# buwantaiji/FermiFlow

Hardware: NVIDIA B200
Metric: VMC walker-updates/s (sample+E_loc+grad) N=20 (higher is better)
Workload: dtype f64

## Files before the change

### fermiflow_b200/csrc/capi.cu

```cuda
#define FF_RADIAL_TABLE_KERNELS
#include "capi_flow.h"
#include "ff_adjoint.cuh"
#include "ff_pgrad_binned.cuh"
#include "ff_misc.cuh"
#include "ff_metro_reg.cuh"
#include "ff_observables.cuh"

namespace ffc {


thread_local char g_err[512] = "";

int fail(int code, const char* fmt, ...) {
    va_list ap;
    va_start(ap, fmt);
    vsnprintf(g_err, sizeof(g_err), fmt, ap);
    va_end(ap);
    return code;
}

int cuda_fail(cudaError_t e, const char* what) {
    return fail((int)e, "%s: %s", what, cudaGetErrorString(e));
}

const char* const kOptNames[] = {
    "no_table", "no_w_balance", "no_rt_cache", "flow_warp_fill", "flow_cta", "flow_big", "eloc_generic", "slater_cta",
    "metropolis_kernel", "adjoint_cta", "pgrad_direct", "pgrad_tile", "pgrad_fixed_range", "adjoint_no_prefetch", "finale_cta",
    "metropolis_no_split"};
static_assert(sizeof(kOptNames) / sizeof(kOptNames[0]) == OPT_COUNT, "one name per option");
std::atomic<int> g_opt[OPT_COUNT];
std::atomic<long long> g_launches{0};

DevInfo dev_info() {
    static thread_local DevInfo di[16];
    int dev = 0;
    cudaGetDevice(&dev);
    DevInfo& d = di[dev & 15];
    if (!d.ok) {
        cudaDeviceGetAttribute(&d.sms, cudaDevAttrMultiProcessorCount, dev);
        cudaDeviceGetAttribute(&d.smem_optin, cudaDevAttrMaxSharedMemoryPerBlockOptin, dev);
        cudaDeviceGetAttribute(&d.smem_sm, cudaDevAttrMaxSharedMemoryPerMultiprocessor, dev);
        cudaDeviceGetAttribute(&d.smem_reserved, cudaDevAttrReservedSharedMemoryPerBlock, dev);
        d.ok = true;
    }
    return d;
}

int check_model(const ff_model* m) {
    if (!m) return fail(-1, "model is null");
    const int n = m->n_up + m->n_dn;
    if (m->n_up < 0 || m->n_dn < 0 || n < 1) return fail(-1, "bad particle numbers %d/%d", m->n_up, m->n_dn);
    if (n > 200) return fail(-1, "n = %d particles exceeds the supported 200", n);
    if (m->H_eta < 1 || m->H_mu < 0) return fail(-1, "bad hidden sizes");
    if (m->nsteps < 1) return fail(-1, "nsteps must be >= 1");
    if (!m->eta_w1 || !m->eta_b1 || !m->eta_w2) return fail(-1, "eta parameters missing");
    if (m->H_mu > 0 && (!m->mu_w1 || !m->mu_b1 || !m->mu_w2)) return fail(-1, "mu parameters missing");
    return 0;
}

int RadialTables::build(const ff_model* m, cudaStream_t stream, ff::FlowArgs& a) {
    a.rt_eta = nullptr; a.rt_mu = nullptr;
    if (opt(OPT_NO_TABLE)) return 0;
    st = stream;
    {
        static thread_local bool pool_ready[16] = {};
        int dev = 0;
        cudaGetDevice(&dev);
        if (!pool_ready[dev & 15]) {
            cudaMemPool_t pool;
            if (cudaDeviceGetDefaultMemPool(&pool, dev) == cudaSuccess) {
                unsigned long long keep = 64ull << 20;
                cudaMemPoolSetAttribute(pool, cudaMemPoolAttrReleaseThreshold, &keep);
            }
            pool_ready[dev & 15] = true;
        }
    }
    const size_t per = ff::radial_table_doubles();
    FF_CUDA(cudaMallocAsync((void**)&buf, 2 * per * sizeof(double), st));
    ff::RadialBuildArgs b{};
    b.w1[0] = m->eta_w1; b.b1[0] = m->eta_b1; b.w2[0] = m->eta_w2; b.H[0] = m->H_eta; b.table[0] = buf;
    b.w1[1] = m->mu_w1; b.b1[1] = m->mu_b1; b.w2[1] = m->mu_w2; b.H[1] = m->H_mu; b.table[1] = m->H_mu > 0 ? buf + per : nullptr;
    ff::radial_table_build_kernel<<<dim3(ff::kRtMaxNodes / 128, 2), 128, 0, st>>>(b);
    FF_LAUNCHED();
    ff::radial_table_check_kernel<<<dim3(1, 2), 128, 0, st>>>(b.table[0], b.table[1]);
    FF_LAUNCHED();
    a.rt_eta = b.table[0]; a.rt_mu = b.table[1];
    return 0;
}

}

using namespace ffc;

extern "C" {

int ff_version(void) { return 200; }

long long ff_launch_count(void) { return g_launches.load(std::memory_order_relaxed); }

int ff_set_option(const char* name, int value) {
    if (!name) return fail(-1, "ff_set_option: null name");
    for (int k = 0; k < OPT_COUNT; ++k)
        if (strcmp(name, kOptNames[k]) == 0) { g_opt[k].store(value, std::memory_order_relaxed); return 0; }
    return fail(-1, "ff_set_option: unknown option '%s'", name);
}
int ff_get_option(const char* name, int* value) {
    if (!name || !value) return fail(-1, "ff_get_option: null argument");
    for (int k = 0; k < OPT_COUNT; ++k)
        if (strcmp(name, kOptNames[k]) == 0) { *value = opt((Opt)k); return 0; }
    return fail(-1, "ff_get_option: unknown option '%s'", name);
}
const char* ff_last_error(void) { return g_err; }

int ff_stash_sizes(const ff_model* m, long long B, long long* ny, long long* nc) {
    if (int e = check_model(m)) return e;
    const long long n = m->n_up + m->n_dn, NS = 4LL * m->nsteps;
    const long long P = n * (n - 1) / 2 + (m->H_mu > 0 ? n : 0);
    if (ny) *ny = B * NS * 2 * n;
    if (nc) *nc = B * NS * P * 3;
    return 0;
}

int ff_cnf_generate(const ff_model* m, const double* z, long long B, int reverse, double* x, void* stream) {
    if (int e = check_model(m)) return e;
    if (B < 0 || (B > 0 && (!z || !x))) return fail(-1, "ff_cnf_generate: null buffer");
    ff::FlowArgs a{};
    int threads; size_t smem;
    if (int e = plan_flow(ff::MODE_V, m, a, threads, smem)) return e;
    a.ta = reverse ? m->t1 : m->t0; a.tb = reverse ? m->t0 : m->t1;
    a.B = B; a.x_in = z; a.y_out = x;
    RadialTables rt;
    if (int e = rt.build(m, (cudaStream_t)stream, a)) return e;
    return launch_flow<ff::MODE_V>(a, threads, smem, (cudaStream_t)stream);
}

int ff_cnf_delta_logp(const ff_model* m, const double* x, long long B, double* z, double* delta_logp,
                      double* stash_y, double* stash_c, void* stream) {
    if (int e = check_model(m)) return e;
    if (B < 0 || (B > 0 && !x)) return fail(-1, "ff_cnf_delta_logp: null input");
    const bool stash = stash_y != nullptr;
    if (stash_c && !stash_y) return fail(-1, "ff_cnf_delta_logp: stash_c needs stash_y");
    ff::FlowArgs a{};
    int threads; size_t smem;
    const int mode = stash ? ff::MODE_STASH : ff::MODE_DIV;
    if (int e = plan_flow(mode, m, a, threads, smem)) return e;
    a.ta = m->t1; a.tb = m->t0;
    a.B = B; a.x_in = x; a.y_out = z; a.delta_out = delta_logp;
    a.stash_y = stash_y; a.stash_c = stash_c;
    RadialTables rt;
    if (int e = rt.build(m, (cudaStream_t)stream, a)) return e;
    return stash ? launch_flow<ff::MODE_STASH>(a, threads, smem, (cudaStream_t)stream)
                 : launch_flow<ff::MODE_DIV>(a, threads, smem, (cudaStream_t)stream);
}

#include "capi_rest.inc"
#ifdef FF_PG_TIMING
extern "C" int ff_debug_pg_cycles(unsigned long long* out, int reset) {
    cudaDeviceSynchronize();
    cudaMemcpyFromSymbol(out, ff::g_pg_cyc, sizeof(unsigned long long) * 160);
    cudaMemcpyFromSymbol(out + 160, ff::g_pg_maxbin, sizeof(unsigned long long) * 4);
    if (reset) { unsigned long long z[160] = {}; cudaMemcpyToSymbol(ff::g_pg_cyc, z, sizeof z); cudaMemcpyToSymbol(ff::g_pg_maxbin, z, 32); }
    return 0;
}
#endif

}
```

### fermiflow_b200/csrc/capi_common.h

```cpp
#pragma once
#include <cmath>
#include <cstdarg>
#include <cstdio>
#include <cstring>
#include <cstdlib>
#include <algorithm>
#include <atomic>
#include <cuda_runtime.h>

#include "../../include/fermiflow_b200.h"

namespace ffc {

int fail(int code, const char* fmt, ...);
int cuda_fail(cudaError_t e, const char* what);

constexpr int FF_FALLBACK = -1000;

enum Opt {
    OPT_NO_TABLE,
    OPT_NO_W_BALANCE,
    OPT_NO_RT_CACHE,
    OPT_FLOW_WARP_FILL,
    OPT_FLOW_CTA,
    OPT_FLOW_BIG,
    OPT_ELOC_GENERIC,
    OPT_SLATER_CTA,
    OPT_METROPOLIS_KERNEL,
    OPT_ADJOINT_CTA,
    OPT_PGRAD_DIRECT,
    OPT_PGRAD_TILE,
    OPT_PGRAD_FIXED_RANGE,
    OPT_ADJOINT_NO_PREFETCH,
    OPT_FINALE_CTA,
    OPT_METROPOLIS_NO_SPLIT,
    OPT_COUNT
};
extern std::atomic<int> g_opt[OPT_COUNT];
inline int opt(Opt o) { return g_opt[o].load(std::memory_order_relaxed); }

#define FF_CUDA(call)                                              \
    do {                                                           \
        cudaError_t e__ = (call);                                  \
        if (e__ != cudaSuccess) return ffc::cuda_fail(e__, #call); \
    } while (0)

extern std::atomic<long long> g_launches;
#define FF_LAUNCHED()                                            \
    do {                                                         \
        ffc::g_launches.fetch_add(1, std::memory_order_relaxed); \
        FF_CUDA(cudaGetLastError());                             \
    } while (0)

struct DevInfo { int sms = 0; int smem_optin = 0; int smem_sm = 0; int smem_reserved = 1024; bool ok = false; };
DevInfo dev_info();
int check_model(const ff_model* m);
inline int even(int x) { return (x + 1) & ~1; }

}
```

### fermiflow_b200/csrc/capi_rest.inc

```

int ff_backflow(const ff_model* m, const double* x, long long B, double* v, double* div, void* stream) {
    if (int e = check_model(m)) return e;
    if (B < 0 || (B > 0 && !x)) return fail(-1, "ff_backflow: null input");
    const DevInfo di = dev_info();
    ff::BackflowArgs a{};
    const int n = m->n_up + m->n_dn;
    a.n = n; a.H_eta = m->H_eta; a.H_mu = m->H_mu;
    a.eta_w1 = m->eta_w1; a.eta_b1 = m->eta_b1; a.eta_w2 = m->eta_w2;
    a.mu_w1 = m->mu_w1; a.mu_b1 = m->mu_b1; a.mu_w2 = m->mu_w2;
    a.B = B; a.x = x; a.v = v; a.div = div;
    a.NP = n * (n - 1) / 2; a.P = a.NP + (m->H_mu > 0 ? n : 0);
    if (a.P < 1) return fail(-1, "ff_backflow: nothing to evaluate");
    if (a.P > 512) return fail(-2, "ff_backflow: n = %d too large", n);
    a.W = 256 / a.P; if (a.W < 1) a.W = 1;
    const int threads = std::max(64, ((a.W * a.P + 31) / 32) * 32);
    const size_t smem = (size_t)(ff::kTabDoubles + 6 * (((m->H_eta + 3) & ~3) + ((m->H_mu + 3) & ~3)) + (long long)a.W * (2 * n + 3 * a.P)) * 8;
    if (smem > (size_t)di.smem_optin) return fail(-2, "ff_backflow: shared memory %zu too large", smem);
    FF_CUDA(cudaFuncSetAttribute(ff::backflow_kernel, cudaFuncAttributeMaxDynamicSharedMemorySize, (int)smem));
    long long grid = std::min<long long>((B + a.W - 1) / a.W, (long long)di.sms * 4);
    if (grid < 1) return 0;
    ff::backflow_kernel<<<(unsigned)grid, threads, smem, (cudaStream_t)stream>>>(a);
    FF_LAUNCHED();
    return 0;
}
// ... 103 lines not shown
        auto launch = [&](auto kernel) -> int {
            FF_CUDA(cudaFuncSetAttribute(kernel, cudaFuncAttributeMaxDynamicSharedMemorySize, (int)smem));
            kernel<<<(unsigned)grid, threads, smem, (cudaStream_t)stream>>>(a);
            FF_LAUNCHED();
            return 0;
        };
        if (smem <= (size_t)di.smem_optin) {
            if (split) {
                if (nsm <= 3) return launch(ff::metropolis_reg_kernel<3, 1>);
                if (nsm <= 6) return launch(ff::metropolis_reg_kernel<6, 1>);
                return launch(ff::metropolis_reg_kernel<10, 1>);
            }
            if (nsm <= 3) return launch(ff::metropolis_reg_kernel<3>);
            if (nsm <= 6) return launch(ff::metropolis_reg_kernel<6>);
            return launch(ff::metropolis_reg_kernel<10>);
        }
    }
    if (nsm <= 16 && mk != 3) {
        const int warps = 8;
        const size_t smem = (size_t)warps * ff::metro_warp_slice(n, nsm) * 8;
        FF_CUDA(cudaFuncSetAttribute(ff::metropolis_warp_kernel, cudaFuncAttributeMaxDynamicSharedMemorySize, (int)smem));
        int occ = 0;
        FF_CUDA(cudaOccupancyMaxActiveBlocksPerMultiprocessor(&occ, ff::metropolis_warp_kernel, 32 * warps, smem));
        if (occ >= 1) {
            const long long grid = std::min<long long>((B + warps - 1) / warps, (long long)di.sms * occ);
            ff::metropolis_warp_kernel<<<(unsigned)grid, 32 * warps, smem, (cudaStream_t)stream>>>(a);
            FF_LAUNCHED();
            return 0;
        }
    }
    int threads = 128;
    size_t per_thread = (size_t)(4 * n + nsm * nsm) * 8;
    while (threads > 32 && per_thread * threads > (size_t)di.smem_optin) threads /= 2;
    double* gs = nullptr;
    size_t smem = per_thread * threads;
    const long long grid = (B + threads - 1) / threads;
    if (smem > (size_t)di.smem_optin) {
        a.use_global = 1;
        smem = (size_t)(4 * n) * 8 * threads;
        FF_CUDA(cudaMallocAsync((void**)&gs, (size_t)nsm * nsm * grid * threads * 8, (cudaStream_t)stream));
        a.gscratch = gs;
    }
    FF_CUDA(cudaFuncSetAttribute(ff::metropolis_kernel, cudaFuncAttributeMaxDynamicSharedMemorySize, (int)smem));
    ff::metropolis_kernel<<<(unsigned)grid, threads, smem, (cudaStream_t)stream>>>(a);
    g_launches.fetch_add(1, std::memory_order_relaxed);
    cudaError_t le = cudaGetLastError();
    if (gs) cudaFreeAsync(gs, (cudaStream_t)stream);
    if (le != cudaSuccess) return cuda_fail(le, "metropolis_kernel");
    return 0;
}

int ff_backward_work_size(const ff_model* m, long long B, long long* n_work) {
    if (int e = check_model(m)) return e;
    const long long n = m->n_up + m->n_dn;
    if (n_work) *n_work = B * 4LL * m->nsteps * 2 * n + 1024LL * 3 * (m->H_eta + m->H_mu)
                          + (long long)ff::pgrad_binned_work_doubles(m->H_eta + m->H_mu);
    return 0;
}

int ff_logp_backward(const ff_model* m, long long B, const double* stash_y, const double* stash_c,
                     const double* gbar_z, const double* gbar_delta, double* grad_x,
                     double* g_eta_w1, double* g_eta_b1, double* g_eta_w2,
                     double* g_mu_w1, double* g_mu_b1, double* g_mu_w2,
                     double* work, void* stream) {
    if (int e = check_model(m)) return e;
    if (B < 0 || (B > 0 && (!stash_y || !gbar_z || !gbar_delta || !work)))
        return fail(-1, "ff_logp_backward: null buffer");
    if ((reinterpret_cast<uintptr_t>(stash_y) | reinterpret_cast<uintptr_t>(work)) & 15)
        return fail(-1, "ff_logp_backward: stash_y and work must be 16-byte aligned (16-byte asynchronous copies)");
    if (B == 0) return 0;
    const DevInfo di = dev_info();
    cudaStream_t st = (cudaStream_t)stream;
    const int n = m->n_up + m->n_dn, D = 2 * n, NP = n * (n - 1) / 2;
    const int P = NP + (m->H_mu > 0 ? n : 0);
    const long long NS = 4LL * m->nsteps;
    const double h = (m->t0 - m->t1) / m->nsteps;
    double* kbar = work;
    double* partial = work + B * NS * D;
    {
        ff::AdjArgs a{};
        a.n = n; a.H_eta = m->H_eta; a.H_mu = m->H_mu; a.nsteps = m->nsteps; a.h = h; a.B = B;
        a.stash_y = stash_y; a.stash_c = stash_c; a.gbar_z = gbar_z; a.gbar_delta = gbar_delta;
        a.kbar = kbar; a.grad_x = grad_x; a.P = P; a.NP = NP; a.D = D;
        a.eta_w1 = m->eta_w1; a.eta_b1 = m->eta_b1; a.eta_w2 = m->eta_w2;
        a.mu_w1 = m->mu_w1; a.mu_b1 = m->mu_b1; a.mu_w2 = m->mu_w2;
        RadialTables rt;
        if (stash_c == nullptr) {
            ff::FlowArgs fa{};
            if (int e = rt.build(m, st, fa)) return e;
            a.rt_eta = fa.rt_eta; a.rt_mu = fa.rt_mu;
        }
        if (P > 512) return fail(-2, "ff_logp_backward: n = %d too large", n);
        a.W = std::max(1, 256 / P);
        const int threads = std::max(64, ((a.W * P + 31) / 32) * 32);
        const size_t smem = (size_t)(2 * ((NP + 7) / 8) + (long long)a.W * (6 * D + 2 * P)) * 8;
        if (smem > (size_t)di.smem_optin) return fail(-2, "ff_logp_backward: shared memory");
        auto launch_adjoint = [&](auto kernel) -> int {
            FF_CUDA(cudaFuncSetAttribute(kernel, cudaFuncAttributeMaxDynamicSharedMemorySize, (int)smem));
            FF_CUDA(cudaFuncSetAttribute(kernel, cudaFuncAttributePreferredSharedMemoryCarveout, (int)cudaSharedmemCarveoutMaxShared));
            int occ = 0;
            FF_CUDA(cudaOccupancyMaxActiveBlocksPerMultiprocessor(&occ, kernel, threads, smem));
            long long grid = std::min<long long>((B + a.W - 1) / a.W, (long long)di.sms * std::max(occ, 1));
            kernel<<<(unsigned)grid, threads, smem, st>>>(a);
            FF_LAUNCHED();
            return 0;
        };
        const int wwarps = 8;
        const size_t wsmem = (size_t)(2 * ((NP + 7) / 8) + (long long)wwarps * ff::adjoint_warp_slice(D, P)) * 8;
        auto launch_adjoint_warp = [&](auto kernel) -> int {
            FF_CUDA(cudaFuncSetAttribute(kernel, cudaFuncAttributeMaxDynamicSharedMemorySize, (int)wsmem));
            FF_CUDA(cudaFuncSetAttribute(kernel, cudaFuncAttributePreferredSharedMemoryCarveout, (int)cudaSharedmemCarveoutMaxShared));
            int occ = 0;
            FF_CUDA(cudaOccupancyMaxActiveBlocksPerMultiprocessor(&occ, kernel, 32 * wwarps, wsmem));
            long long grid = std::min<long long>((B + wwarps - 1) / wwarps, (long long)di.sms * std::max(occ, 1));
            kernel<<<(unsigned)grid, 32 * wwarps, wsmem, st>>>(a);
            FF_LAUNCHED();
            return 0;
        };
        if (wsmem <= (size_t)di.smem_optin / 2 && !opt(OPT_ADJOINT_CTA)) {
            const bool pf = !opt(OPT_ADJOINT_NO_PREFETCH);
            if (int e = (stash_c == nullptr) ? (pf ? launch_adjoint_warp(ff::adjoint_warp_kernel<true, true>) : launch_adjoint_warp(ff::adjoint_warp_kernel<true, false>))
                                             : (pf ? launch_adjoint_warp(ff::adjoint_warp_kernel<false, true>) : launch_adjoint_warp(ff::adjoint_warp_kernel<false, false>))) return e;
        } else if (int e = (stash_c == nullptr) ? launch_adjoint(ff::adjoint_kernel<true>) : launch_adjoint(ff::adjoint_kernel<false>)) return e;
    }
    const bool want_params = g_eta_w1 || g_eta_b1 || g_eta_w2 || g_mu_w1 || g_mu_b1 || g_mu_w2;
    if (!want_params) return 0;
    const double* binned_hdr = nullptr;
    if (!opt(OPT_PGRAD_DIRECT) && m->H_eta + m->H_mu <= ff::kPgMaxBins && n <= 255) {
        ff::PGradBinArgs b{};
        b.n = n; b.H_eta = m->H_eta; b.H_mu = m->H_mu; b.nsteps = m->nsteps; b.h = h; b.B = B;
        b.stash_y = stash_y; b.kbar = kbar; b.gbar_delta = gbar_delta;
        b.eta_w1 = m->eta_w1; b.eta_b1 = m->eta_b1; b.eta_w2 = m->eta_w2;
        b.mu_w1 = m->mu_w1; b.mu_b1 = m->mu_b1; b.mu_w2 = m->mu_w2;
        b.work = partial + 1024LL * 3 * (m->H_eta + m->H_mu);
        b.NP = NP; b.D = D;
        b.ge_w1 = g_eta_w1; b.ge_b1 = g_eta_b1; b.ge_w2 = g_eta_w2; b.gm_w1 = g_mu_w1; b.gm_b1 = g_mu_b1; b.gm_w2 = g_mu_w2;
        int R = opt(OPT_PGRAD_TILE) > 0 ? opt(OPT_PGRAD_TILE) : 32;
        auto smem_of = [&](int r) { return ff::pgrad_binned_smem_bytes(r, P, D, NP); };
        while (R > 1 && (smem_of(R) > (size_t)di.smem_optin || (long long)R * P > 65000)) R -= (R > 8 ? 4 : 1);
        if (smem_of(R) <= (size_t)di.smem_optin && (long long)R * P <= 65000) {
            b.R = R;
            const size_t smem = smem_of(R);
            const long long nrec_all = B * NS;
            if (!opt(OPT_PGRAD_FIXED_RANGE) && NP > 0 && NP <= 16384) {
                int* hist = reinterpret_cast<int*>(b.work + ff::pgrad_binned_zeroed_doubles(m->H_eta + m->H_mu));
                FF_CUDA(cudaMemsetAsync(hist, 0, ff::kPgHist * sizeof(int), st));
                const long long stride = std::max<long long>(1, nrec_all / 65536) | 1;
                const long long rows = (nrec_all + stride - 1) / stride;
                ff::pgrad_hist_kernel<<<(unsigned)std::min<long long>(rows, 4LL * di.sms), 256, 0, st>>>(b, stride);
                FF_LAUNCHED();
            } else {
                FF_CUDA(cudaMemsetAsync(b.work + ff::pgrad_binned_zeroed_doubles(m->H_eta + m->H_mu), 0, ff::kPgHist * sizeof(int), st));
            }
            ff::pgrad_bins_setup_kernel<<<32, 256, 0, st>>>(b);
            FF_LAUNCHED();
            FF_CUDA(cudaFuncSetAttribute(ff::pgrad_binned_kernel, cudaFuncAttributeMaxDynamicSharedMemorySize, (int)smem));
            int bocc = 0;
            FF_CUDA(cudaOccupancyMaxActiveBlocksPerMultiprocessor(&bocc, ff::pgrad_binned_kernel, ff::kPgMaxBins, smem));
            const long long ntiles = ((B + R - 1) / R) * NS;
            const long long grid = std::min<long long>(ntiles, (long long)di.sms * std::max(bocc, 1));
            ff::pgrad_binned_kernel<<<(unsigned)grid, ff::kPgMaxBins, smem, st>>>(b);
            FF_LAUNCHED();
            ff::pgrad_binned_finish_kernel<<<m->H_eta + m->H_mu, 256, 0, st>>>(b);
            FF_LAUNCHED();
            binned_hdr = b.work;
        }
    }
    {
        ff::PGradArgs a{};
        a.binned_hdr = binned_hdr;
        a.n = n; a.H_eta = m->H_eta; a.H_mu = m->H_mu; a.nsteps = m->nsteps; a.h = h; a.B = B;
        a.stash_y = stash_y; a.kbar = kbar; a.gbar_delta = gbar_delta;
        a.eta_w1 = m->eta_w1; a.eta_b1 = m->eta_b1; a.mu_w1 = m->mu_w1; a.mu_b1 = m->mu_b1;
        a.partial = partial; a.NP = NP; a.D = D;
        if (m->H_eta > 512 || m->H_eta + m->H_mu > 512)
            return fail(-2, "ff_logp_backward: hidden sizes %d + %d exceed 512 threads", m->H_eta, m->H_mu);
        int S_e = 1, S_m = m->H_mu > 0 ? 1 : 0;
        if (NP == 0) { S_e = 1; }
        for (int se = 1; se <= 512; ++se) {
            int sm = 0;
            if (m->H_mu > 0) sm = std::max(1, (int)((long long)se * n / std::max(NP, 1)));
            if (m->H_eta * se + m->H_mu * sm > 512) break;
            S_e = se; S_m = sm;
        }
        a.S_e = S_e; a.S_m = S_m;
        const int used = m->H_eta * S_e + m->H_mu * S_m;
        const int threads = std::max(64, ((used + 31) / 32) * 32);
        int R = 8;
        auto smem_of = [&](int r) {
            long long d = ff::kTabDoubles + (long long)r * 2 * D + ((r + 1) & ~1) + (long long)r * NP * 4 + (long long)r * n * 4 + 2 * ((NP + 7) / 8) + 2;
            d = std::max<long long>(d, ff::kTabDoubles + 3LL * threads + 8);
            return (size_t)d * 8;
        };
        while (R > 1 && smem_of(R) > (size_t)96 * 1024) R /= 2;
        if (smem_of(R) > (size_t)di.smem_optin) return fail(-2, "ff_logp_backward: shared memory (pgrad)");
        a.R = R;
        const size_t smem = smem_of(R);
        FF_CUDA(cudaFuncSetAttribute(ff::pgrad_kernel, cudaFuncAttributeMaxDynamicSharedMemorySize, (int)smem));
        FF_CUDA(cudaFuncSetAttribute(ff::pgrad_kernel, cudaFuncAttributePreferredSharedMemoryCarveout, (int)cudaSharedmemCarveoutMaxShared));
        int occ = 0;
        FF_CUDA(cudaOccupancyMaxActiveBlocksPerMultiprocessor(&occ, ff::pgrad_kernel, threads, smem));
        const long long nrec = B * NS;
        long long grid = std::min<long long>((nrec + R - 1) / R, std::min<long long>(1024, (long long)di.sms * std::max(occ, 1)));
        ff::pgrad_kernel<<<(unsigned)grid, threads, smem, st>>>(a);
        FF_LAUNCHED();
        ff::pgrad_finish_kernel<<<1, 256, 0, st>>>(partial, (int)grid, m->H_eta, m->H_mu, m->eta_w2, m->mu_w2,
                                                   g_eta_w1, g_eta_b1, g_eta_w2, g_mu_w1, g_mu_b1, g_mu_w2, binned_hdr);
        FF_LAUNCHED();
    }
    return 0;
}

int ff_potential(const double* x, long long B, int n, double Z, int harmonic, double* V, void* stream) {
    if (n < 1 || B < 0 || (B > 0 && (!x || !V))) return fail(-1, "ff_potential: bad arguments");
    if (B == 0) return 0;
    ff::potential_kernel<<<(unsigned)((B + 127) / 128), 128, 0, (cudaStream_t)stream>>>(x, B, n, Z, harmonic, V);
    FF_LAUNCHED();
    return 0;
}

int ff_observables(const double* x, long long B, int n_up, int n_dn, const ff_obs_grid* g,
                   unsigned long long* counts, long long n_counts, void* stream) {
    using namespace ff;
    const long long n = (long long)n_up + n_dn;
    if (n_up < 0 || n_dn < 0 || n < 1) return fail(-1, "ff_observables: bad particle numbers %d/%d", n_up, n_dn);
    if (!g) return fail(-1, "ff_observables: null grid");
    if (g->n_xy < 0 || g->n_r < 0 || g->n_rot < 0)
        return fail(-1, "ff_observables: negative bin count (n_xy %d, n_r %d, n_rot %d)", g->n_xy, g->n_r, g->n_rot);
    if ((g->n_xy > 0 || g->n_rot > 0) && !(g->extent > 0 && std::isfinite(g->extent)))
        return fail(-1, "ff_observables: extent must be positive and finite (got %g)", g->extent);
    if (g->n_r > 0 && !(g->r_max > 0 && std::isfinite(g->r_max)))
        return fail(-1, "ff_observables: r_max must be positive and finite (got %g)", g->r_max);
    const long long nb[OBS_SECTIONS] = {g->n_xy, g->n_r, g->n_r, g->n_rot};
    const long long nch[OBS_SECTIONS] = {2, 2, 3, 2};
    const long long sq[OBS_SECTIONS] = {1, 0, 0, 1};
    const long long items[OBS_SECTIONS] = {n, n, n * (n - 1) / 2, n * (n - 1)};
    const char* const names[OBS_SECTIONS] = {"density", "radial", "separation", "rotated"};
    long long bins[OBS_SECTIONS], goff[OBS_SECTIONS], total = 0;
    for (int s = 0; s < OBS_SECTIONS; ++s) {
        bins[s] = nch[s] * (sq[s] ? nb[s] * nb[s] : nb[s]);
        goff[s] = total;
        total += bins[s];
    }
    if (n_counts != total + kObsOutside)
        return fail(-1, "ff_observables: n_counts = %lld, the layout of this grid has %lld", n_counts, total + kObsOutside);
    if (B < 0 || (B > 0 && (!x || !counts))) return fail(-1, "ff_observables: bad walker count or null buffer");
    if (B == 0) return 0;
    const DevInfo di = dev_info();
    int on = 0;
    long long all_bins = 0;
    for (int s = 0; s < OBS_SECTIONS; ++s) {
        if (nb[s] == 0) continue;
        on |= 1 << s;
        all_bins += bins[s];
        const long long bytes = (bins[s] + kObsOutside) * 4;
        if (bytes > di.smem_optin)
            return fail(-1, "ff_observables: the %s section needs %lld bytes of shared memory, more than the %d bytes a "
                        "block can have on this device", names[s], bytes, di.smem_optin);
    }
    const bool together = (all_bins + kObsOutside) * 4 <= di.smem_optin;
    for (int s0 = 0; s0 < OBS_SECTIONS; ++s0) {
        const int mask = together ? on : (on & (1 << s0));
        if (!mask || (together && s0 > 0)) continue;
        ObsArgs a{};
        a.x = x; a.B = B; a.n = (int)n; a.n_up = n_up; a.mask = mask; a.counts = counts; a.outside_off = total;
        long long sb = 0, it = 0;
        for (int s = 0; s < OBS_SECTIONS; ++s) {
            const bool in = mask >> s & 1;
            a.nb[s] = (int)nb[s];
            a.goff[s] = goff[s];
            a.soff[s] = (int)sb;
            a.first[s] = (int)it;
            if (in) { sb += bins[s]; it += items[s]; }
        }
        a.first[OBS_SECTIONS] = (int)it;
        a.lo[OBS_DENSITY] = a.lo[OBS_ROTATED] = -g->extent;
        a.s[OBS_DENSITY] = g->n_xy / (2.0 * g->extent);
        a.s[OBS_ROTATED] = g->n_rot / (2.0 * g->extent);
        a.lo[OBS_RADIAL] = a.lo[OBS_SEPARATION] = 0.0;
        a.s[OBS_RADIAL] = a.s[OBS_SEPARATION] = g->n_r / g->r_max;
        a.sbins = (int)sb;
        if (it == 0) continue;
        const long long chunk_max = (0xFFFFFFFFLL - kObsThreads) / it;
        if (chunk_max < 1) return fail(-1, "ff_observables: n = %lld particles give too many pairs per walker", n);
        a.items = (unsigned)it;
        const size_t smem = (size_t)(sb + kObsOutside) * 4;
        FF_CUDA(cudaFuncSetAttribute(observables_kernel, cudaFuncAttributeMaxDynamicSharedMemorySize, (int)smem));
        int occ = 0;
        FF_CUDA(cudaOccupancyMaxActiveBlocksPerMultiprocessor(&occ, observables_kernel, kObsThreads, smem));
        const long long ctas = (long long)di.sms * std::max(occ, 1);
        a.chunk = std::min(chunk_max, (B + ctas - 1) / ctas);
        const long long grid = std::min(ctas, (B + a.chunk - 1) / a.chunk);
        observables_kernel<<<(unsigned)grid, kObsThreads, smem, (cudaStream_t)stream>>>(a);
        FF_LAUNCHED();
    }
    return 0;
}

int ff_occupation_sample(const double* logits, int S, const double* uniforms, long long B,
                         int* state, int* counts, double* cdf_work, void* stream) {
    if (S < 1 || B < 0 || !logits || !counts || !cdf_work || (B > 0 && !uniforms)) return fail(-1, "ff_occupation_sample: bad arguments");
    cudaStream_t st = (cudaStream_t)stream;
    ff::occupation_cdf_kernel<<<1, 256, 0, st>>>(logits, S, cdf_work, counts);
    FF_LAUNCHED();
    if (B == 0) return 0;
    ff::occupation_search_kernel<<<(unsigned)((B + 255) / 256), 256, 0, st>>>(cdf_work, S, uniforms, B, counts);
    FF_LAUNCHED();
    if (state) {
        ff::occupation_fill_kernel<<<(unsigned)std::min(S, 1024), 256, 0, st>>>(counts, S, B, state);
        FF_LAUNCHED();
    }
    return 0;
}

int ff_fp64_peak(int iters, double* flops_host, void* stream) {
// ... 56 lines not shown
```

### fermiflow_b200/csrc/ff_pgrad_binned.cuh

```cuda
#pragma once
#include "ff_adjoint.cuh"
#include "ff_radial_table.cuh"

namespace ff {

#ifndef FF_PG_BINS
#define FF_PG_BINS 640
#endif
constexpr int kPgMaxBins = FF_PG_BINS;
constexpr int kPgMom = 12;
constexpr double kPgSpacing = 0.25;
constexpr double kPgDmax = 24.0;
constexpr double kPgDmaxMu = 12.0;
constexpr double kPgMaxDelta = 0.25;
constexpr int kPgHdr = 16;
constexpr int kPgHist = 512;
constexpr double kPgQuantile = 0.999;
__host__ __device__ inline size_t pgrad_binned_zeroed_doubles(int Ht) { return kPgHdr + (size_t)kPgMaxBins * 2 * kPgMom + 3 * (size_t)Ht; }
__host__ __device__ inline size_t pgrad_binned_work_doubles(int Ht) { return pgrad_binned_zeroed_doubles(Ht) + kPgHist / 2; }

struct PGradBinArgs {
    int n, H_eta, H_mu, nsteps;
    double h;
    long long B;
    const double *stash_y, *kbar, *gbar_delta;
    const double *eta_w1, *eta_b1, *eta_w2, *mu_w1, *mu_b1, *mu_w2;
    double* work;
    int R, NP, D;
    double *ge_w1, *ge_b1, *ge_w2, *gm_w1, *gm_b1, *gm_w2;
};

__global__ void __launch_bounds__(256) pgrad_hist_kernel(const PGradBinArgs a, long long stride) {
    __shared__ int hist[kPgHist];
    __shared__ unsigned char pi[32768 / 2], pj[32768 / 2];
    const int tid = threadIdx.x, n = a.n, D = a.D, NP = a.NP;
    for (int k = tid; k < kPgHist; k += blockDim.x) hist[k] = 0;
    for (int p = tid; p < NP; p += blockDim.x) {
        int i = 0, rem = p;
        while (rem >= n - 1 - i) { rem -= n - 1 - i; ++i; }
        pi[p] = (unsigned char)i; pj[p] = (unsigned char)(i + 1 + rem);
    }
    __syncthreads();
    const long long nrec = a.B * 4LL * a.nsteps;
    for (long long row = (long long)blockIdx.x * stride; row < nrec; row += (long long)gridDim.x * stride) {
        const double* y = a.stash_y + row * D;
        for (int p = tid; p < NP; p += blockDim.x) {
            const int i = pi[p], j = pj[p];
            const double rx = y[2 * i] - y[2 * j], ry = y[2 * i + 1] - y[2 * j + 1];
            const double d = sqrt(fma(rx, rx, ry * ry));
            const double kf = d * (kPgHist / kPgDmax);
            atomicAdd(&hist[kf < (double)(kPgHist - 1) ? (int)kf : kPgHist - 1], 1);
        }
    }
    __syncthreads();
    int* gh = reinterpret_cast<int*>(a.work + pgrad_binned_zeroed_doubles(a.H_eta + a.H_mu));
    for (int k = tid; k < kPgHist; k += blockDim.x) if (hist[k]) atomicAdd(gh + k, hist[k]);
}

__global__ void __launch_bounds__(256) pgrad_bins_setup_kernel(const PGradBinArgs a) {
    __shared__ double red[256];
    const int Ht = a.H_eta + a.H_mu;
    double* hdr = a.work;
    const size_t total = pgrad_binned_zeroed_doubles(Ht);
    for (size_t i = kPgHdr + (size_t)blockIdx.x * blockDim.x + threadIdx.x; i < total; i += (size_t)gridDim.x * blockDim.x) a.work[i] = 0.0;
    if (blockIdx.x != 0) return;
    double wmx[2];
    for (int f = 0; f < 2; ++f) {
        const int H = f ? a.H_mu : a.H_eta;
        const double* w1 = f ? a.mu_w1 : a.eta_w1;
        double wm = 0.0;
        for (int hh = threadIdx.x; hh < H; hh += blockDim.x) wm = fmax(wm, fabs(w1[hh]));
        red[threadIdx.x] = wm;
        __syncthreads();
        for (int o = 128; o > 0; o >>= 1) { if (threadIdx.x < o) red[threadIdx.x] = fmax(red[threadIdx.x], red[threadIdx.x + o]); __syncthreads(); }
        wmx[f] = red[0];
        __syncthreads();
    }
    if (threadIdx.x == 0) {
        const double dm_max = fmin(kPgMaxDelta, kPgSpacing / fmax(wmx[1], 1e-300));
        const double de_max = fmin(kPgMaxDelta, kPgSpacing / fmax(wmx[0], 1e-300));
        const double nbm = a.H_mu > 0 ? ceil(kPgDmaxMu / dm_max) + 1.0 : 0.0;
        double range = kPgDmax;
        bool far = false;
        {
            const int* gh = reinterpret_cast<const int*>(a.work + total);
            long long all = 0, cum = 0;
            for (int k = 0; k < kPgHist; ++k) all += gh[k];
            if (all > 0) {
                int q = 0;
                for (; q < kPgHist; ++q) { cum += gh[q]; if ((double)cum >= kPgQuantile * (double)all) break; }
                range = fmin(kPgDmax, fmax(1.0, (q + 2) * (kPgDmax / kPgHist)));
                far = (double)gh[kPgHist - 1] > 4.0 * (1.0 - kPgQuantile) * (double)all;
            }
        }
        const double nbe_min = ceil(range / de_max) + 1.0;
        const bool ok = !far && isfinite(wmx[0]) && isfinite(wmx[1]) && nbm + nbe_min <= (double)kPgMaxBins;
        double nbm_f = nbm, dm = dm_max, nbe = nbe_min, de = de_max;
        if (ok) {
            if (a.H_mu > 0) {
                const double rmu = fmin(kPgDmaxMu, range);
                nbm_f = fmin(ceil(2.0 * rmu / dm_max) + 1.0, (double)kPgMaxBins - nbe_min);
                nbm_f = fmax(nbm_f, ceil(rmu / dm_max) + 1.0);
                if (nbm_f + nbe_min <= (double)kPgMaxBins) dm = rmu / (nbm_f - 1.0);
                else { nbm_f = nbm; dm = dm_max; }
            }
            nbe = (double)kPgMaxBins - nbm_f;
            de = range / (nbe - 1.0);
        }
        hdr[0] = 1.0 / de; hdr[1] = de; hdr[2] = nbe;
        hdr[3] = 1.0 / dm; hdr[4] = dm; hdr[5] = nbm_f;
        hdr[6] = ok ? 1.0 : 0.0; hdr[7] = range;
    }
}

#ifdef FF_PG_TIMING
__device__ unsigned long long g_pg_cyc[20][8];
__device__ unsigned long long g_pg_maxbin[4];
#define PGT(seg) do { if (lane == 0) { const long long t_ = clock64(); atomicAdd(&g_pg_cyc[warp][seg], (unsigned long long)(t_ - tprev)); tprev = t_; } } while (0)
#else
#define PGT(seg) do { } while (0)
#endif

constexpr int kPgCap = 40;
__host__ __device__ inline size_t pgrad_binned_smem_bytes(int R, int P, int D, int NP) {
    const size_t REC = (size_t)R * P;
    return 8 * ((size_t)kTabDoubles + 2 * (size_t)R * 2 * D + 2 * ((R + 1) & ~1) + 3 * REC)
           + 4 * ((size_t)kPgMaxBins + 8)
           + 2 * ((size_t)kPgMaxBins * kPgCap + ((REC + 3) & ~(size_t)3))
           + 2 * (size_t)((NP + 7) & ~7) + 64;
}

__global__ void __launch_bounds__(kPgMaxBins, kPgMaxBins <= 320 ? 2 : 1) pgrad_binned_kernel(const PGradBinArgs a) {
    extern __shared__ __align__(16) double smem[];
    const double* hdr = a.work;
    if (hdr[6] == 0.0) return;
    const int tid = threadIdx.x, T = blockDim.x, lane = tid & 31, warp = tid >> 5;
    const int n = a.n, D = a.D, NP = a.NP, R = a.R;
    const int P = NP + (a.H_mu > 0 ? n : 0);
    const int NS = 4 * a.nsteps, Ht = a.H_eta + a.H_mu;
    const double inv_de = hdr[0], de = hdr[1], inv_dm = hdr[3], dm = hdr[4];
    const int nb_e = (int)hdr[2], nb_m = (int)hdr[5], nbins = nb_e + nb_m;
    const int REC = R * P;
    (void)warp;
    double* tab = smem;
    double* ysk0 = tab + kTabDoubles;
    double* kdl0 = ysk0 + (size_t)2 * R * 2 * D;
    double* rec_t = kdl0 + 2 * ((R + 1) & ~1);
    double* rec_A = rec_t + REC;
    double* rec_B = rec_A + REC;
    int* cur = reinterpret_cast<int*>(rec_B + REC);
    int* ovf_counts = cur + kPgMaxBins;
    unsigned short* slots = reinterpret_cast<unsigned short*>(ovf_counts + 8);
    unsigned short* ovf = slots + (size_t)kPgMaxBins * kPgCap;
    unsigned char* pair_i = reinterpret_cast<unsigned char*>(ovf + ((REC + 3) & ~3));
    unsigned char* pair_j = pair_i + ((NP + 7) & ~7);

    fill_exp_table(tab);
    const double* tabl = tab + (tid & 15);
    for (int p = tid; p < NP; p += T) {
        int i = 0, rem = p;
        while (rem >= n - 1 - i) { rem -= n - 1 - i; ++i; }
        pair_i[p] = (unsigned char)i;
        pair_j[p] = (unsigned char)(i + 1 + rem);
    }
    const int dir_slices = max(1, T / max(Ht, 1)), dir_slice = tid / max(Ht, 1), dir_u = tid - dir_slice * max(Ht, 1);
    const bool dir_on = dir_slice < dir_slices && Ht > 0;
    const bool dir_eta = dir_u < a.H_eta;
    const int dir_h = dir_eta ? dir_u : dir_u - a.H_eta;
    const double dw1 = dir_on ? (dir_eta ? a.eta_w1 : a.mu_w1)[dir_h] : 0.0;
    const double db1 = dir_on ? (dir_eta ? a.eta_b1 : a.mu_b1)[dir_h] : 0.0;
    double s_w2 = 0.0, s_b1 = 0.0, s_w1 = 0.0;
    double MA[kPgMom], MB[kPgMom];
#pragma unroll
    for (int m = 0; m < kPgMom; ++m) { MA[m] = 0.0; MB[m] = 0.0; }
    const int my_bin = tid;

#ifdef FF_PG_TIMING
    long long tprev = clock64();
#endif
    const long long wblocks = (a.B + R - 1) / R, ntiles = wblocks * NS;
    auto tile_rows = [&](long long tix, long long& w0, int& stage) -> int {
        const long long wb = tix / NS;
        w0 = wb * R; stage = (int)(tix - wb * NS);
        return (int)min((long long)R, a.B - w0);
    };
    auto fetch_tile = [&](long long tix, int buf) {
        if (tix >= ntiles) return;
        long long w0; int stage;
        const int nr = tile_rows(tix, w0, stage);
        double* yb = ysk0 + (size_t)buf * R * 2 * D;
        const int D2 = D, Dh = D >> 1;
        int r = tid / D2, e = tid - r * D2;
        const int dr = T / D2, de_ = T - dr * D2;
        for (int g = tid; g < nr * D2; g += T) {
            const long long rr = (w0 + r) * NS + stage;
            const double* src = (e < Dh) ? a.stash_y + rr * D + 2 * e : a.kbar + rr * D + 2 * (e - Dh);
            asm volatile("cp.async.cg.shared.global [%0], [%1], 16;" ::"r"((unsigned)__cvta_generic_to_shared(yb + 2 * g)), "l"(src));
            r += dr; e += de_;
            if (e >= D2) { e -= D2; ++r; }
        }
        asm volatile("cp.async.commit_group;" ::: "memory");
        double* kb = kdl0 + buf * ((R + 1) & ~1);
        const int sb = stage & 3;
        const double wgt = a.h * ((sb == 0 || sb == 3) ? 0.125 : 0.375);
        for (int q = tid; q < nr; q += T) kb[q] = a.gbar_delta[w0 + q] * wgt;
    };
    if (tid < kPgMaxBins) cur[tid] = 0;
    if (tid < 2) ovf_counts[tid] = 0;
    fetch_tile((long long)blockIdx.x, 0);
    int buf = 0;
    for (long long tix = blockIdx.x; tix < ntiles; tix += gridDim.x, buf ^= 1) {
        long long w0_; int stage_;
        const int nr = tile_rows(tix, w0_, stage_);
        const double* ysk = ysk0 + (size_t)buf * R * 2 * D;
        const double* kdl = kdl0 + buf * ((R + 1) & ~1);
        PGT(0);
        asm volatile("cp.async.wait_group 0;" ::: "memory");
        __syncthreads();
        PGT(1);
        int* ovf_count = ovf_counts + buf;
        if (tid == 0) ovf_counts[buf ^ 1] = 0;
        {
            int r = tid / P, p = tid - r * P;
            const int dr = T / P, dp = T - dr * P;
            for (int g = tid; g < nr * P; g += T) {
                const double* y = ysk + (size_t)r * 2 * D;
                const double* k = y + D;
                const double kd = kdl[r];
                double rx, ry, kx, ky, A, Bc, d;
                const bool pr = p < NP;
                if (pr) {
                    const int i = pair_i[p], j = pair_j[p];
                    const double2 yi = *reinterpret_cast<const double2*>(y + 2 * i), yj = *reinterpret_cast<const double2*>(y + 2 * j);
                    const double2 ki = *reinterpret_cast<const double2*>(k + 2 * i), kj = *reinterpret_cast<const double2*>(k + 2 * j);
                    rx = yi.x - yj.x; ry = yi.y - yj.y; kx = ki.x - kj.x; ky = ki.y - kj.y;
                    { const double d2 = fma(rx, rx, ry * ry); d = d2 * rsqrt(d2); }
                    A = fma(kx, rx, ky * ry) - 4.0 * kd; Bc = -2.0 * kd * d;
                } else {
                    const int i = p - NP;
                    const double2 yi = *reinterpret_cast<const double2*>(y + 2 * i), ki = *reinterpret_cast<const double2*>(k + 2 * i);
                    rx = yi.x; ry = yi.y; kx = ki.x; ky = ki.y;
                    { const double d2 = fma(rx, rx, ry * ry); d = d2 * rsqrt(d2); }
                    A = fma(kx, rx, ky * ry) - 2.0 * kd; Bc = -kd * d;
                }
                const double kf = rint(d * (pr ? inv_de : inv_dm));
                const int nb = pr ? nb_e : nb_m;
                rec_A[g] = A; rec_B[g] = Bc;
                bool placed = false;
                if (kf < (double)nb) {
                    const int bin = (int)kf + (pr ? 0 : nb_e);
                    const int pos = atomicAdd(&cur[bin], 1);
                    if (pos < kPgCap) {
                        rec_t[g] = fma(-kf, pr ? de : dm, d);
                        slots[bin * kPgCap + pos] = (unsigned short)g;
                        placed = true;
                    }
                }
                if (!placed) {
                    rec_t[g] = d;
                    ovf[atomicAdd(ovf_count, 1)] = (unsigned short)g;
                }
                r += dr; p += dp;
                if (p >= P) { p -= P; ++r; }
            }
        }
        PGT(2);
        __syncthreads();
        PGT(3);
        fetch_tile(tix + gridDim.x, buf ^ 1);
        PGT(4);
#ifdef FF_PG_TIMING
        {
            unsigned long long c = my_bin < nbins ? (unsigned long long)min(cur[my_bin], kPgCap) : 0;
            for (int o = 16; o > 0; o >>= 1) { unsigned long long v = __shfl_xor_sync(0xffffffffu, c, o); c = v > c ? v : c; }
            if (lane == 0) { atomicAdd(&g_pg_maxbin[3], c); atomicMax(&g_pg_maxbin[0], c); if (warp == 0) atomicAdd(&g_pg_maxbin[2], 1ull); }
            tprev = clock64();
        }
#endif
        if (my_bin < nbins) {
            const unsigned short* sl = slots + my_bin * kPgCap;
            const int p1 = min(cur[my_bin], kPgCap);
            cur[my_bin] = 0;
            int p = 0;
            for (; p + 2 <= p1; p += 2) {
                const int g0 = sl[p], g1 = sl[p + 1];
                const double t0 = rec_t[g0], A0 = rec_A[g0], B0 = rec_B[g0];
                const double t1 = rec_t[g1], A1 = rec_A[g1], B1 = rec_B[g1];
                double pw0 = 1.0, pw1 = 1.0;
#pragma unroll
                for (int m = 0; m < kPgMom; ++m) {
                    MA[m] = fma(A0, pw0, MA[m]); MB[m] = fma(B0, pw0, MB[m]);
                    MA[m] = fma(A1, pw1, MA[m]); MB[m] = fma(B1, pw1, MB[m]);
                    pw0 *= t0; pw1 *= t1;
                }
            }
            if (p < p1) {
                const int g = sl[p];
                const double t = rec_t[g], A = rec_A[g], Bc = rec_B[g];
                double pw = 1.0;
#pragma unroll
                for (int m = 0; m < kPgMom; ++m) { MA[m] = fma(A, pw, MA[m]); MB[m] = fma(Bc, pw, MB[m]); pw *= t; }
            }
        }
        PGT(5);
        const int novf = *ovf_count;
        if (novf > 0 && dir_on) {
            for (int q = dir_slice; q < novf; q += dir_slices) {
                const int g = ovf[q];
                const int p = g % P;
                if ((p < NP) != dir_eta) continue;
                const double d = rec_t[g], A = rec_A[g], Bc = rec_B[g];
                const double s = sigmoid_fast(fma(dw1, d, db1), tabl);
                const double s1 = fma(-s, s, s);
                const double s2 = s1 * fma(-2.0, s, 1.0);
                const double Bw = Bc * dw1;
                const double X = fma(A, s1, Bw * s2);
                s_w2 = fma(A, s, fma(Bw, s1, s_w2));
                s_b1 += X;
                s_w1 = fma(d, X, fma(Bc, s1, s_w1));
            }
        }
    }
    double* mom = a.work + kPgHdr;
    double* direct = mom + (size_t)kPgMaxBins * 2 * kPgMom;
    if (my_bin < nbins) {
#pragma unroll
        for (int m = 0; m < kPgMom; ++m) {
            atomicAdd(mom + (size_t)my_bin * 2 * kPgMom + m, MA[m]);
            atomicAdd(mom + (size_t)my_bin * 2 * kPgMom + kPgMom + m, MB[m]);
        }
    }
    if (dir_on && (s_w2 != 0.0 || s_b1 != 0.0 || s_w1 != 0.0)) {
        atomicAdd(direct + 3 * dir_u, s_w2); atomicAdd(direct + 3 * dir_u + 1, s_b1); atomicAdd(direct + 3 * dir_u + 2, s_w1);
    }
}

__global__ void __launch_bounds__(256) pgrad_binned_finish_kernel(const PGradBinArgs a) {
    __shared__ double tab[kTabDoubles];
    __shared__ double red[3][256];
    const double* hdr = a.work;
    if (hdr[6] == 0.0) return;
    fill_exp_table(tab);
    __syncthreads();
    const double* tabl = tab + (threadIdx.x & 15);
    const int hh = blockIdx.x;
    const bool e = hh < a.H_eta;
    const int hi = e ? hh : hh - a.H_eta;
    const double w1 = (e ? a.eta_w1 : a.mu_w1)[hi], b1 = (e ? a.eta_b1 : a.mu_b1)[hi], w2 = (e ? a.eta_w2 : a.mu_w2)[hi];
    const double delta = hdr[e ? 1 : 4];
    const int nb = (int)hdr[e ? 2 : 5], bin0 = e ? 0 : (int)hdr[2];
    const double* mom = a.work + kPgHdr;
    const double* direct = mom + (size_t)kPgMaxBins * 2 * kPgMom;
    double S2 = 0.0, Sb = 0.0, S1 = 0.0;
    for (int k = threadIdx.x; k < nb; k += blockDim.x) {
        const double dk = k * delta;
        const double s = sigmoid_fast(fma(w1, dk, b1), tabl);
        double c[kPgMom];
        double wp = 1.0;
#pragma unroll
        for (int m = 0; m < kPgMom; ++m) {
            const double* p = c_sigpoly + c_sigpoly_off[m];
            double v = p[m + 1];
#pragma unroll
            for (int q = m; q >= 0; --q) v = fma(v, s, p[q]);
            c[m] = wp * c_inv_fact[m] * v;
            wp *= w1;
        }
        const double* MA = mom + (size_t)(bin0 + k) * 2 * kPgMom;
        const double* MB = MA + kPgMom;
        double gA = 0.0, gB = 0.0;
#pragma unroll
        for (int m = 0; m < kPgMom; ++m) gA = fma(MA[m], c[m], gA);
#pragma unroll
        for (int m = 0; m + 1 < kPgMom; ++m) gB = fma(MB[m], (m + 1) * c[m + 1], gB);
        S2 += gA + gB;
        double Q[kPgMom - 1];
        wp = 1.0;
#pragma unroll
        for (int m = 0; m + 1 < kPgMom; ++m) {
            const double* p = c_sigpoly + c_sigpoly_off[m + 1];
            double v = p[m + 2];
#pragma unroll
            for (int q = m + 1; q >= 0; --q) v = fma(v, s, p[q]);
            Q[m] = wp * c_inv_fact[m] * v;
            wp *= w1;
        }
        double X0 = 0.0, X1 = 0.0, Bq = 0.0;
#pragma unroll
        for (int m = 0; m + 1 < kPgMom; ++m) {
            X0 = fma(MA[m], Q[m], X0);
            X1 = fma(MA[m + 1], Q[m], X1);
            Bq = fma(MB[m], Q[m], Bq);
        }
#pragma unroll
        for (int m = 0; m + 2 < kPgMom; ++m) {
            X0 = fma(MB[m], (m + 1) * Q[m + 1], X0);
            X1 = fma(MB[m + 1], (m + 1) * Q[m + 1], X1);
        }
        Sb += X0;
        S1 += fma(dk, X0, X1) + Bq;
    }
    red[0][threadIdx.x] = S2; red[1][threadIdx.x] = Sb; red[2][threadIdx.x] = S1;
    __syncthreads();
    for (int o = 128; o > 0; o >>= 1) {
        if (threadIdx.x < o) for (int q = 0; q < 3; ++q) red[q][threadIdx.x] += red[q][threadIdx.x + o];
        __syncthreads();
    }
    if (threadIdx.x == 0) {
        const double s2 = red[0][0] + direct[3 * hh], sb = red[1][0] + direct[3 * hh + 1], s1 = red[2][0] + direct[3 * hh + 2];
        double* gw2 = e ? a.ge_w2 : a.gm_w2; double* gb1 = e ? a.ge_b1 : a.gm_b1; double* gw1 = e ? a.ge_w1 : a.gm_w1;
        if (gw2) gw2[hi] += s2;
        if (gb1) gb1[hi] += w2 * sb;
        if (gw1) gw1[hi] += w2 * s1;
    }
}

}
```

Baseline: 647,600.

## Pick Taylor moment order adaptively per histogram bin in binned param-gradient

The setup kernel now chooses a truncation order (7, 8, 10 or 12) for the binned Taylor-moment expansion, based on the largest w1 times bin width. The binned kernel is templated on the order and launched once per candidate order, and each launch exits early unless it matches the chosen one. The bin walk and the finish kernel then only accumulate and read that many moments. This cuts FMA work and register pressure when the weights are small, at the cost of three extra near-empty launches and lower expansion accuracy near the chosen bound.

```diff
diff --git a/fermiflow_b200/csrc/capi.cu b/fermiflow_b200/csrc/capi.cu
--- a/fermiflow_b200/csrc/capi.cu
+++ b/fermiflow_b200/csrc/capi.cu
@@ -26,7 +26,7 @@
 const char* const kOptNames[] = {
     "no_table", "no_w_balance", "no_rt_cache", "flow_warp_fill", "flow_cta", "flow_big", "eloc_generic", "slater_cta",
     "metropolis_kernel", "adjoint_cta", "pgrad_direct", "pgrad_tile", "pgrad_fixed_range", "adjoint_no_prefetch", "finale_cta",
-    "metropolis_no_split"};
+    "metropolis_no_split", "pgrad_order"};
 static_assert(sizeof(kOptNames) / sizeof(kOptNames[0]) == OPT_COUNT, "one name per option");
 std::atomic<int> g_opt[OPT_COUNT];
 std::atomic<long long> g_launches{0};
@@ -156,11 +156,13 @@
 #include "capi_rest.inc"
 #ifdef FF_PG_TIMING
 extern "C" int ff_debug_pg_cycles(unsigned long long* out, int reset) {
+    constexpr int ncyc = ff::kPgWarps * 8;
+    if (!out) return ff::kPgWarps;
     cudaDeviceSynchronize();
-    cudaMemcpyFromSymbol(out, ff::g_pg_cyc, sizeof(unsigned long long) * 160);
-    cudaMemcpyFromSymbol(out + 160, ff::g_pg_maxbin, sizeof(unsigned long long) * 4);
-    if (reset) { unsigned long long z[160] = {}; cudaMemcpyToSymbol(ff::g_pg_cyc, z, sizeof z); cudaMemcpyToSymbol(ff::g_pg_maxbin, z, 32); }
-    return 0;
+    cudaMemcpyFromSymbol(out, ff::g_pg_cyc, sizeof(unsigned long long) * ncyc);
+    cudaMemcpyFromSymbol(out + ncyc, ff::g_pg_maxbin, sizeof(unsigned long long) * 4);
+    if (reset) { unsigned long long z[ncyc] = {}; cudaMemcpyToSymbol(ff::g_pg_cyc, z, sizeof z); cudaMemcpyToSymbol(ff::g_pg_maxbin, z, 32); }
+    return ff::kPgWarps;
 }
 #endif
 
diff --git a/fermiflow_b200/csrc/capi_common.h b/fermiflow_b200/csrc/capi_common.h
--- a/fermiflow_b200/csrc/capi_common.h
+++ b/fermiflow_b200/csrc/capi_common.h
@@ -34,6 +34,7 @@
     OPT_ADJOINT_NO_PREFETCH,
     OPT_FINALE_CTA,
     OPT_METROPOLIS_NO_SPLIT,
+    OPT_PGRAD_ORDER,
     OPT_COUNT
 };
 extern std::atomic<int> g_opt[OPT_COUNT];
diff --git a/fermiflow_b200/csrc/capi_rest.inc b/fermiflow_b200/csrc/capi_rest.inc
--- a/fermiflow_b200/csrc/capi_rest.inc
+++ b/fermiflow_b200/csrc/capi_rest.inc
@@ -279,15 +279,24 @@
             } else {
                 FF_CUDA(cudaMemsetAsync(b.work + ff::pgrad_binned_zeroed_doubles(m->H_eta + m->H_mu), 0, ff::kPgHist * sizeof(int), st));
             }
+            b.min_order = opt(OPT_PGRAD_ORDER);
             ff::pgrad_bins_setup_kernel<<<32, 256, 0, st>>>(b);
             FF_LAUNCHED();
-            FF_CUDA(cudaFuncSetAttribute(ff::pgrad_binned_kernel, cudaFuncAttributeMaxDynamicSharedMemorySize, (int)smem));
-            int bocc = 0;
-            FF_CUDA(cudaOccupancyMaxActiveBlocksPerMultiprocessor(&bocc, ff::pgrad_binned_kernel, ff::kPgMaxBins, smem));
-            const long long ntiles = ((B + R - 1) / R) * NS;
-            const long long grid = std::min<long long>(ntiles, (long long)di.sms * std::max(bocc, 1));
-            ff::pgrad_binned_kernel<<<(unsigned)grid, ff::kPgMaxBins, smem, st>>>(b);
-            FF_LAUNCHED();
+            auto launch_binned = [&](auto kernel) -> int {
+                FF_CUDA(cudaFuncSetAttribute(kernel, cudaFuncAttributeMaxDynamicSharedMemorySize, (int)smem));
+                int bocc = 0;
+                FF_CUDA(cudaOccupancyMaxActiveBlocksPerMultiprocessor(&bocc, kernel, ff::kPgMaxBins, smem));
+                const long long ntiles = ((B + R - 1) / R) * NS;
+                const long long grid = std::min<long long>(ntiles, (long long)di.sms * std::max(bocc, 1));
+                kernel<<<(unsigned)grid, ff::kPgMaxBins, smem, st>>>(b);
+                FF_LAUNCHED();
+                return 0;
+            };
+            static_assert(ff::kPgNumOrders == 4 && ff::kPgOrders[3] == ff::kPgMom, "one launch per order of kPgOrders");
+            if (int e = launch_binned(ff::pgrad_binned_kernel<ff::kPgOrders[0]>)) return e;
+            if (int e = launch_binned(ff::pgrad_binned_kernel<ff::kPgOrders[1]>)) return e;
+            if (int e = launch_binned(ff::pgrad_binned_kernel<ff::kPgOrders[2]>)) return e;
+            if (int e = launch_binned(ff::pgrad_binned_kernel<ff::kPgOrders[3]>)) return e;
             ff::pgrad_binned_finish_kernel<<<m->H_eta + m->H_mu, 256, 0, st>>>(b);
             FF_LAUNCHED();
             binned_hdr = b.work;
diff --git a/fermiflow_b200/csrc/ff_pgrad_binned.cuh b/fermiflow_b200/csrc/ff_pgrad_binned.cuh
--- a/fermiflow_b200/csrc/ff_pgrad_binned.cuh
+++ b/fermiflow_b200/csrc/ff_pgrad_binned.cuh
@@ -9,6 +9,8 @@
 #endif
 constexpr int kPgMaxBins = FF_PG_BINS;
 constexpr int kPgMom = 12;
+constexpr int kPgOrders[] = {7, 8, 10, 12};
+constexpr int kPgNumOrders = sizeof(kPgOrders) / sizeof(kPgOrders[0]);
 constexpr double kPgSpacing = 0.25;
 constexpr double kPgDmax = 24.0;
 constexpr double kPgDmaxMu = 12.0;
@@ -27,6 +29,7 @@
     const double *eta_w1, *eta_b1, *eta_w2, *mu_w1, *mu_b1, *mu_w2;
     double* work;
     int R, NP, D;
+    int min_order;
     double *ge_w1, *ge_b1, *ge_w2, *gm_w1, *gm_b1, *gm_w2;
 };
 
@@ -55,6 +58,18 @@
     __syncthreads();
     int* gh = reinterpret_cast<int*>(a.work + pgrad_binned_zeroed_doubles(a.H_eta + a.H_mu));
     for (int k = tid; k < kPgHist; k += blockDim.x) if (hist[k]) atomicAdd(gh + k, hist[k]);
+}
+
+template <int k = 0>
+__device__ inline int pgrad_moment_order(double x, int min_order) {
+    if constexpr (k == kPgNumOrders) {
+        return kPgMom;
+    } else {
+        constexpr int M = kPgOrders[k];
+        const double c = 0.5 / 3.14159265358979323846;
+        if (M >= min_order && pow(x * c, M) <= pow(kPgSpacing * c, kPgMom)) return M;
+        return pgrad_moment_order<k + 1>(x, min_order);
+    }
 }
 
 __global__ void __launch_bounds__(256) pgrad_bins_setup_kernel(const PGradBinArgs a) {
@@ -110,11 +125,15 @@
         hdr[0] = 1.0 / de; hdr[1] = de; hdr[2] = nbe;
         hdr[3] = 1.0 / dm; hdr[4] = dm; hdr[5] = nbm_f;
         hdr[6] = ok ? 1.0 : 0.0; hdr[7] = range;
+        const int me = pgrad_moment_order(wmx[0] * de, a.min_order);
+        hdr[8] = me;
+        hdr[9] = a.H_mu > 0 ? pgrad_moment_order(wmx[1] * dm, a.min_order) : me;
     }
 }
 
 #ifdef FF_PG_TIMING
-__device__ unsigned long long g_pg_cyc[20][8];
+constexpr int kPgWarps = kPgMaxBins / 32;
+__device__ unsigned long long g_pg_cyc[kPgWarps][8];
 __device__ unsigned long long g_pg_maxbin[4];
 #define PGT(seg) do { if (lane == 0) { const long long t_ = clock64(); atomicAdd(&g_pg_cyc[warp][seg], (unsigned long long)(t_ - tprev)); tprev = t_; } } while (0)
 #else
@@ -130,10 +149,53 @@
            + 2 * (size_t)((NP + 7) & ~7) + 64;
 }
 
+template <int K, int M>
+__device__ __forceinline__ void pgrad_bin_walk(double (&MA)[M], double (&MB)[M], const unsigned short* sl, int p1,
+                                               const double* rec_t, const double* rec_A, const double* rec_B) {
+    static_assert(K <= M, "order beyond the register arrays");
+    int p = 0;
+    for (; p + 2 <= p1; p += 2) {
+        const int g0 = sl[p], g1 = sl[p + 1];
+        const double t0 = rec_t[g0], A0 = rec_A[g0], B0 = rec_B[g0];
+        const double t1 = rec_t[g1], A1 = rec_A[g1], B1 = rec_B[g1];
+        double pw0 = 1.0, pw1 = 1.0;
+#pragma unroll
+        for (int m = 0; m < K; ++m) {
+            MA[m] = fma(A0, pw0, MA[m]); MB[m] = fma(B0, pw0, MB[m]);
+            MA[m] = fma(A1, pw1, MA[m]); MB[m] = fma(B1, pw1, MB[m]);
+            pw0 *= t0; pw1 *= t1;
+        }
+    }
+    if (p < p1) {
+        const int g = sl[p];
+        const double t = rec_t[g], A = rec_A[g], Bc = rec_B[g];
+        double pw = 1.0;
+#pragma unroll
+        for (int m = 0; m < K; ++m) { MA[m] = fma(A, pw, MA[m]); MB[m] = fma(Bc, pw, MB[m]); pw *= t; }
+    }
+}
+
+constexpr int pgrad_lower_order(int K) {
+    int r = 0;
+    for (int k = 0; k < kPgNumOrders; ++k) if (kPgOrders[k] < K) r = kPgOrders[k];
+    return r;
+}
+
+template <int M, int K = M>
+__device__ __forceinline__ void pgrad_bin_walk_order(int k, double (&MA)[M], double (&MB)[M], const unsigned short* sl, int p1,
+                                                     const double* rec_t, const double* rec_A, const double* rec_B) {
+    if constexpr (K > 0) {
+        if (k == K) pgrad_bin_walk<K>(MA, MB, sl, p1, rec_t, rec_A, rec_B);
+        else pgrad_bin_walk_order<M, pgrad_lower_order(K)>(k, MA, MB, sl, p1, rec_t, rec_A, rec_B);
+    }
+}
+
+template <int M>
 __global__ void __launch_bounds__(kPgMaxBins, kPgMaxBins <= 320 ? 2 : 1) pgrad_binned_kernel(const PGradBinArgs a) {
     extern __shared__ __align__(16) double smem[];
     const double* hdr = a.work;
     if (hdr[6] == 0.0) return;
+    if ((int)fmax(hdr[8], hdr[9]) != M) return;
     const int tid = threadIdx.x, T = blockDim.x, lane = tid & 31, warp = tid >> 5;
     const int n = a.n, D = a.D, NP = a.NP, R = a.R;
     const int P = NP + (a.H_mu > 0 ? n : 0);
@@ -156,7 +218,6 @@
     unsigned char* pair_j = pair_i + ((NP + 7) & ~7);
 
     fill_exp_table(tab);
-    const double* tabl = tab + (tid & 15);
     for (int p = tid; p < NP; p += T) {
         int i = 0, rem = p;
         while (rem >= n - 1 - i) { rem -= n - 1 - i; ++i; }
@@ -167,13 +228,12 @@
     const bool dir_on = dir_slice < dir_slices && Ht > 0;
     const bool dir_eta = dir_u < a.H_eta;
     const int dir_h = dir_eta ? dir_u : dir_u - a.H_eta;
-    const double dw1 = dir_on ? (dir_eta ? a.eta_w1 : a.mu_w1)[dir_h] : 0.0;
-    const double db1 = dir_on ? (dir_eta ? a.eta_b1 : a.mu_b1)[dir_h] : 0.0;
     double s_w2 = 0.0, s_b1 = 0.0, s_w1 = 0.0;
-    double MA[kPgMom], MB[kPgMom];
-#pragma unroll
-    for (int m = 0; m < kPgMom; ++m) { MA[m] = 0.0; MB[m] = 0.0; }
+    double MA[M], MB[M];
+#pragma unroll
+    for (int m = 0; m < M; ++m) { MA[m] = 0.0; MB[m] = 0.0; }
     const int my_bin = tid;
+    const int my_order = (int)hdr[my_bin < nb_e ? 8 : 9];
 
 #ifdef FF_PG_TIMING
     long long tprev = clock64();
@@ -278,33 +338,15 @@
         }
 #endif
         if (my_bin < nbins) {
-            const unsigned short* sl = slots + my_bin * kPgCap;
             const int p1 = min(cur[my_bin], kPgCap);
             cur[my_bin] = 0;
-            int p = 0;
-            for (; p + 2 <= p1; p += 2) {
-                const int g0 = sl[p], g1 = sl[p + 1];
-                const double t0 = rec_t[g0], A0 = rec_A[g0], B0 = rec_B[g0];
-                const double t1 = rec_t[g1], A1 = rec_A[g1], B1 = rec_B[g1];
-                double pw0 = 1.0, pw1 = 1.0;
-#pragma unroll
-                for (int m = 0; m < kPgMom; ++m) {
-                    MA[m] = fma(A0, pw0, MA[m]); MB[m] = fma(B0, pw0, MB[m]);
-                    MA[m] = fma(A1, pw1, MA[m]); MB[m] = fma(B1, pw1, MB[m]);
-                    pw0 *= t0; pw1 *= t1;
-                }
-            }
-            if (p < p1) {
-                const int g = sl[p];
-                const double t = rec_t[g], A = rec_A[g], Bc = rec_B[g];
-                double pw = 1.0;
-#pragma unroll
-                for (int m = 0; m < kPgMom; ++m) { MA[m] = fma(A, pw, MA[m]); MB[m] = fma(Bc, pw, MB[m]); pw *= t; }
-            }
+            pgrad_bin_walk_order<M>(my_order, MA, MB, slots + my_bin * kPgCap, p1, rec_t, rec_A, rec_B);
         }
         PGT(5);
         const int novf = *ovf_count;
         if (novf > 0 && dir_on) {
+            const double dw1 = (dir_eta ? a.eta_w1 : a.mu_w1)[dir_h], db1 = (dir_eta ? a.eta_b1 : a.mu_b1)[dir_h];
+            const double* tabl = tab + (tid & 15);
             for (int q = dir_slice; q < novf; q += dir_slices) {
                 const int g = ovf[q];
                 const int p = g % P;
@@ -325,7 +367,8 @@
     double* direct = mom + (size_t)kPgMaxBins * 2 * kPgMom;
     if (my_bin < nbins) {
 #pragma unroll
-        for (int m = 0; m < kPgMom; ++m) {
+        for (int m = 0; m < M; ++m) {
+            if (m >= my_order) break;
             atomicAdd(mom + (size_t)my_bin * 2 * kPgMom + m, MA[m]);
             atomicAdd(mom + (size_t)my_bin * 2 * kPgMom + kPgMom + m, MB[m]);
         }
@@ -349,6 +392,7 @@
     const double w1 = (e ? a.eta_w1 : a.mu_w1)[hi], b1 = (e ? a.eta_b1 : a.mu_b1)[hi], w2 = (e ? a.eta_w2 : a.mu_w2)[hi];
     const double delta = hdr[e ? 1 : 4];
     const int nb = (int)hdr[e ? 2 : 5], bin0 = e ? 0 : (int)hdr[2];
+    const int M = (int)hdr[e ? 8 : 9];
     const double* mom = a.work + kPgHdr;
     const double* direct = mom + (size_t)kPgMaxBins * 2 * kPgMom;
     double S2 = 0.0, Sb = 0.0, S1 = 0.0;
@@ -370,9 +414,9 @@
         const double* MB = MA + kPgMom;
         double gA = 0.0, gB = 0.0;
 #pragma unroll
-        for (int m = 0; m < kPgMom; ++m) gA = fma(MA[m], c[m], gA);
-#pragma unroll
-        for (int m = 0; m + 1 < kPgMom; ++m) gB = fma(MB[m], (m + 1) * c[m + 1], gB);
+        for (int m = 0; m < kPgMom; ++m) if (m < M) gA = fma(MA[m], c[m], gA);
+#pragma unroll
+        for (int m = 0; m + 1 < kPgMom; ++m) if (m + 1 < M) gB = fma(MB[m], (m + 1) * c[m + 1], gB);
         S2 += gA + gB;
         double Q[kPgMom - 1];
         wp = 1.0;
@@ -388,12 +432,14 @@
         double X0 = 0.0, X1 = 0.0, Bq = 0.0;
 #pragma unroll
         for (int m = 0; m + 1 < kPgMom; ++m) {
+            if (m + 1 >= M) break;
             X0 = fma(MA[m], Q[m], X0);
             X1 = fma(MA[m + 1], Q[m], X1);
             Bq = fma(MB[m], Q[m], Bq);
         }
 #pragma unroll
         for (int m = 0; m + 2 < kPgMom; ++m) {
+            if (m + 2 >= M) break;
             X0 = fma(MB[m], (m + 1) * Q[m + 1], X0);
             X1 = fma(MB[m + 1], (m + 1) * Q[m + 1], X1);
         }
```

Result: faster. 661,600 (median of 6 runs) (+2.2%).
